# crowsonkb/style_transfer

Measured on AMD Instinct MI355X. Metric: tile-iterations/sec, VGG-19 2048px/1024-tile (fwd+bwd, Gram/content losses, regularizers, Adam step), higher is better.
Workload: dtype f32 (fp16x2-split MFMA, fp32 accumulate)

## Files before the change

style_transfer_amd/csrc/common.h:

```cpp
#pragma once

#include <hip/hip_runtime.h>

#include <vector>

#include <cstdarg>
#include <cstdio>
#include <functional>
#include <string>

#include "stx.h"

namespace stx {

constexpr float kEps = 1.1920928955078125e-07f;

void set_error(const char *fmt, ...);

const char *sw_env(const char *name);
void sw_reread();

#define STX_HIP(call)                                                                       \
    do {                                                                                    \
        hipError_t err__ = (call);                                                          \
// ... 175 lines not shown
    unsigned char *pool_codes;
    int skip_y = 0;
    unsigned char *out_codes = nullptr;
    unsigned char *in_codes = nullptr;
    const unsigned char *mask_codes = nullptr;
    long long *clock_out = nullptr;
    int item_base = 0;
    const unsigned *x_amax = nullptr;
    unsigned *y_amax = nullptr;
    const unsigned char *pin_codes = nullptr;
    int pin_mode = 0, pin_mask = 0;
#ifdef STX_EXPERIMENT_BF3
    int vp_rows = 0, vp_tp = 0;
#endif
};

bool conv_first_usable(int K, int M, int ksize);
int conv_first_workgroups(int H, int W);
int conv_first_launch(hipStream_t s, const float *x, const float *w_caffe, const float *bias, float *y,
                      int K, int H, int W, int relu, float *gram_partials, unsigned *y_amax = nullptr);

ConvConfig wino2_config(int geometry = 0);
int wino2_pick_geometry(int H, int W);
size_t wino2_packed_floats(int K, int M);
int wino2_pack_weights(hipStream_t s, const float *w_caffe, int Mo, int Ko, int transpose_flip,
                       float *packed);
int wino2_launch(hipStream_t s, const ConvConfig &cfg, const ConvProblem &p, int ksplit);
bool wino2_fuses_pool(const ConvProblem &p);
bool wino2_uses_relu_codes(const ConvProblem &p, int ksplit);
bool wino2_writes_out_codes(const ConvConfig &cfg, const ConvProblem &p);
int wino2_splitk_factor(const ConvConfig &cfg, const ConvProblem &p);
struct Wino2Tail { int items, slices; };
Wino2Tail wino2_tail_split(const ConvConfig &cfg, const ConvProblem &p);
int wino2_max_slices(const ConvConfig &cfg, const ConvProblem &p);

constexpr int kAmaxSlots = 64;
ConvConfig h2_config(int mb, int pb = 1);
ConvConfig h2_pick_config(const ConvProblem &p);
bool h2_usable(const ConvProblem &p);
size_t h2_packed_floats(int K, int M);
int h2_pack_weights(hipStream_t s, const float *w_caffe, int Mo, int Ko, int transpose_flip, float *packed);
int h2_launch(hipStream_t s, const ConvConfig &cfg, const ConvProblem &p, int ksplit);
int h2_splitk_factor(const ConvConfig &cfg, const ConvProblem &p);
bool h2_fuses_pool(const ConvProblem &p);
bool h2_takes_pooled_input(const ConvConfig &cfg, const ConvProblem &p);
int absmax_launch(hipStream_t s, const float *x, size_t n, unsigned *slots);

size_t conv_small_packed_floats(int K);
int conv_small_pack(hipStream_t s, const float *w_caffe, int Mo, int Ko, int transpose_flip,
                    float *packed);
int conv_small_launch(hipStream_t s, const float *x, const float *packed, float *y,
                      const float *mask, int K, int M, int H, int W);

bool conv_h2_enabled();
struct ConvTuner { int device; hipStream_t stream; hipEvent_t ev0, ev1; std::function<int(const ConvConfig &, const float **)> bank; };
int conv_choose(const ConvProblem &p, bool winograd, const ConvTuner *tuner, ConvConfig *out);
struct ConvBank { int key; size_t floats; std::function<int(hipStream_t, const float *w_caffe, float *packed)> pack; };
ConvBank conv_bank(const ConvConfig &cfg, int dir, int Mo, int Ko, int ksize);
ConvBank conv_small_bank(int Mo, int Ko);
int conv_dispatch(hipStream_t s, const ConvConfig &cfg, const ConvProblem &p, double *flop_algorithmic,
                  double *flop_issued);
int conv_splitk_factor(const ConvConfig &cfg, const ConvProblem &p);
size_t conv_splitk_floats(const ConvConfig &cfg, const ConvProblem &p);
bool conv_takes_clock(const ConvConfig &cfg);
bool conv_fuses_pool(const ConvConfig &cfg, const ConvProblem &p);
bool conv_writes_pool_codes(const ConvConfig &cfg);
bool conv_reads_x_amax(const ConvConfig &cfg);
bool conv_leaves_y_amax(const ConvConfig &cfg);
bool conv_takes_inject(const ConvConfig &cfg);
bool conv_takes_pooled_input(const ConvConfig &cfg, const ConvProblem &p);
bool conv_uses_relu_codes(const ConvConfig &cfg, const ConvProblem &p, int ksplit);
bool conv_writes_out_codes(const ConvConfig &cfg, const ConvProblem &p, int ksplit);

int pool_forward_launch(hipStream_t s, const float *x, int C, int H, int W, int mode, float *y,
                        unsigned char *codes = nullptr);
int pool_backward_codes_launch(hipStream_t s, const float *dy, const unsigned char *codes, int C,
                               int H, int W, int mode, bool relu_mask, float *dx);
int pool_backward_launch(hipStream_t s, const float *dy, const float *x, int C, int H, int W,
                         int mode, bool relu_mask, float *dx);

struct GramPlan {
    int C, HW, splits, tiles;
    int parts;
    size_t partial_floats;
};
GramPlan gram_plan(int C, int HW);
bool gram_h2_usable(const float *feat, int C, int HW);
int gram_partials_launch(hipStream_t s, const float *feat, const GramPlan &plan, float *partials,
                         const unsigned *f_amax = nullptr);
int gram_finish_blocks(const GramPlan &plan);
int gram_finish_launch(hipStream_t s, const float *partials, const GramPlan &plan, float *gram_out,
                       const float *target, float *dsym, float *sumsq, unsigned short *pieces = nullptr,
                       const unsigned *f_amax = nullptr, float *block_out = nullptr);

size_t symm_pieces_elems(int C);
int symm_num_workgroups(int C, int HW);
bool symm_bf3_usable(const float *feat, const float *out, int C, int HW);
bool symm_h2_usable(const float *feat, const float *out, int C, int HW);
int symm_h2_launch(hipStream_t s, const float *feat, const float *dsym, const unsigned *d_amax, int n_damax,
                   const unsigned *f_amax, float *out, float *partials, int C, int HW);
int symm_bf3_launch(hipStream_t s, const float *feat, const float *dsym, unsigned short *pieces,
                    bool pieces_ready, float *out, float *partials, int C, int HW);

#ifdef __HIPCC__
__device__ __forceinline__ int content_origin_y(const ContentWindow &w) { return w.oy - w.sy; }
__device__ __forceinline__ int content_origin_x(const ContentWindow &w) { return w.ox - w.sx; }
__device__ __forceinline__ size_t content_index(const ContentWindow &w, int c, int y, int x) {
    int yy = (content_origin_y(w) + y) % w.ch;
    int xx = (content_origin_x(w) + x) % w.cw;
    if (yy < 0) yy += w.ch;
    if (xx < 0) xx += w.cw;
    return ((size_t)c * w.ch + yy) * w.cw + xx;
}
#endif

struct SumJob {
    const float *src;
    int n;
    float *dst;
};
int sum_jobs_launch(hipStream_t s, const SumJob *jobs, int n_jobs);
int content_sums_launch(hipStream_t s, const float *feat, const float *content,
                        const ContentWindow &win, float *sums , std::vector<SumJob> *defer = nullptr);
int inject_style_launch(hipStream_t s, float *diff, const float *sgrad, size_t n,
                        const float *abs_sum, float coef, bool accumulate, unsigned *y_amax = nullptr);
int inject_content_launch(hipStream_t s, float *diff, const float *feat, const float *content,
                          const ContentWindow &win, const float *sums, float coef, bool accumulate,
                          unsigned *y_amax = nullptr);
int relu_inplace_launch(hipStream_t s, float *x, size_t n);
int sum_partials_launch(hipStream_t s, const float *partials, int n, float *out);
int sum_partials2_launch(hipStream_t s, const float *a, int na, float *out_a, const float *b, int nb,
                         float *out_b);

constexpr int kMaskParts = 1024;
constexpr int kMaskSgradParts = 2048;
int mask_map_launch(hipStream_t s, const float *mask, int H, int W, int scale, float *out);
int mask_apply_launch(hipStream_t s, const float *feat, const float *map, const ContentWindow &win, float *fm,
                      float *m2_partials, int *n_parts);
int mask_target_launch(hipStream_t s, const float *gs, int C, const float *m2_partials, int n_parts, int HW,
                       float *out, float *a_out);
int mask_sgrad_launch(hipStream_t s, float *sgrad, const float *map, const ContentWindow &win, const float *a,
                      float *partials, int *n_parts);

constexpr int kContentMaskParts = 1024;
int content_mask_mean_launch(hipStream_t s, const float *map, const ContentWindow &win, float *a_out);
int content_mask_term_launch(hipStream_t s, const float *feat, const float *content, const float *map,
                             const ContentWindow &win, const float *a, float *sgrad, float *partials,
                             int *n_parts);

constexpr int kStatSlice = 16384;
constexpr float kStatEps = 1e-5f;
int stat_slices(int HW);
size_t stat_scratch_floats(int C, int HW);
int stat_partials_launch(hipStream_t s, const float *feat, int C, int HW, float *partials);
int stat_finish_launch(hipStream_t s, const float *partials, int C, int HW, const float *MU, const float *SD,
                       float *table, float *e_out, float *mean_out, float *sd_out);
int stat_grad_launch(hipStream_t s, const float *feat, int C, int HW, const float *table, float *sgrad,
                     float *abs_partials, int *n_parts);

constexpr int kNnfmQ = 128, kNnfmB = 128, kNnfmK = 32, kNnfmMaxSlices = 64;
constexpr int kNnfmMaxK = 4;
struct NnfmPlan {
    int q_blocks, b_blocks, slices, blocks_per_slice;
};
NnfmPlan nnfm_plan(int n, int M);
size_t nnfm_pieces_floats(int rows, int C);
// ... 99 lines not shown
```

style_transfer_amd/csrc/gram.hip:

```cpp

#include <algorithm>
#include <cstdlib>
#include <cstring>

#include "bf16x3.h"
#include "common.h"
#include "f16x2.h"

namespace stx {

typedef float f32x16 __attribute__((ext_vector_type(16)));

constexpr int kGT = 64;
constexpr int kGP = 64;
constexpr int kGLd = kGP + 1;

GramPlan gram_plan(int C, int HW) {
    GramPlan p;
    p.C = C;
    p.HW = HW;
    const int T = ceil_div(C, kGT);
    p.tiles = T * (T + 1) / 2;
    int target = 512, min_stages = 8;
    if (const char *env = sw_env("STX_GRAM_WGS")) target = std::max(1, atoi(env));
    if (const char *env = sw_env("STX_GRAM_MIN_STAGES")) min_stages = std::max(1, atoi(env));
    int splits = std::max(1, target / p.tiles);
    splits = std::min(splits, ceil_div(HW, min_stages * kGP));
    splits = std::max(splits, 1);
    p.splits = splits;
    p.parts = 1;
    p.partial_floats = (size_t)p.splits * p.parts * p.tiles * kGT * kGT;
    return p;
}

__device__ __forceinline__ void tile_coords(int tile, int &ti, int &tj) {
    int r = (int)((sqrtf(8.f * tile + 1.f) - 1.f) * 0.5f);
    while ((r + 1) * (r + 2) / 2 <= tile) ++r;
    while (r * (r + 1) / 2 > tile) --r;
    ti = r;
    tj = tile - r * (r + 1) / 2;
}

template <bool VEC4>
__global__ __launch_bounds__(256, 2) void gram_partial_kernel(const float *__restrict__ F, int C,
                                                              int HW, int tiles, int slice,
                                                              int parts,
                                                              float *__restrict__ partials) {
    __shared__ float At[kGT * kGLd];
    __shared__ float Bt[kGT * kGLd];
    const int tid = threadIdx.x, lane = tid & 63;
    const int wave = __builtin_amdgcn_readfirstlane(tid >> 6);
    const int l31 = lane & 31, half = lane >> 5;
    const int tile = blockIdx.x % tiles, split = blockIdx.x / tiles;
    int ti, tj;
    tile_coords(tile, ti, tj);
    const bool diag = ti == tj;
    const int p_begin = split * slice;
    const int p_end = min(HW, p_begin + slice);
    const int bi = wave >> 1, bj = wave & 1;

    f32x16 acc;
#pragma unroll
    for (int r = 0; r < 16; ++r) acc[r] = 0.f;

    float ra[16], rb[16];
    auto load = [&](int p0) {
        if (VEC4) {
#pragma unroll
            for (int n = 0; n < 4; ++n) {
                const int e = tid + 256 * n;
                const int ch = e >> 4, px = p0 + (e & 15) * 4;
                const int ca = ti * kGT + ch, cb = tj * kGT + ch;
                const bool okp = px < p_end;
                const bool oka = okp && ca < C, okb = okp && cb < C && !diag;
                const float4 va = *reinterpret_cast<const float4 *>(F + (oka ? (size_t)ca * HW + px : 0));
                const float4 vb = *reinterpret_cast<const float4 *>(F + (okb ? (size_t)cb * HW + px : 0));
                ra[4 * n + 0] = oka ? va.x : 0.f;
                ra[4 * n + 1] = oka ? va.y : 0.f;
                ra[4 * n + 2] = oka ? va.z : 0.f;
                ra[4 * n + 3] = oka ? va.w : 0.f;
                rb[4 * n + 0] = okb ? vb.x : 0.f;
                rb[4 * n + 1] = okb ? vb.y : 0.f;
                rb[4 * n + 2] = okb ? vb.z : 0.f;
                rb[4 * n + 3] = okb ? vb.w : 0.f;
            }
        } else {
#pragma unroll
            for (int n = 0; n < 16; ++n) {
                const int e = tid + 256 * n;
                const int ch = e >> 6, px = p0 + (e & 63);
                const int ca = ti * kGT + ch, cb = tj * kGT + ch;
                const bool okp = px < p_end;
                const bool oka = okp && ca < C, okb = okp && cb < C && !diag;
                const float va = F[oka ? (size_t)ca * HW + px : 0];
                const float vb = F[okb ? (size_t)cb * HW + px : 0];
                ra[n] = oka ? va : 0.f;
                rb[n] = okb ? vb : 0.f;
            }
        }
    };
    auto store = [&]() {
        if (VEC4) {
#pragma unroll
            for (int n = 0; n < 4; ++n) {
                const int e = tid + 256 * n;
                const int ch = e >> 4, px = (e & 15) * 4;
#pragma unroll
                for (int k = 0; k < 4; ++k) {
                    At[ch * kGLd + px + k] = ra[4 * n + k];
                    if (!diag) Bt[ch * kGLd + px + k] = rb[4 * n + k];
                }
// ... 372 lines not shown
        }
    };
    auto store = [&](int p0, int buf) {
        float *At = lds + buf * kStageFloats, *Bt = At + kGT * kGLdW;
#pragma unroll
        for (int n = 0; n < 4; ++n) {
            const int rem = p_end - (p0 + ((tid + 256 * n) & 15) * 4);
            u32x4g va = ra[n], vb = rb[n];
            if (rem < 4) {
                va.x = rem > 0 ? va.x : 0u, va.y = rem > 1 ? va.y : 0u, va.z = rem > 2 ? va.z : 0u, va.w = 0u;
                vb.x = rem > 0 ? vb.x : 0u, vb.y = rem > 1 ? vb.y : 0u, vb.z = rem > 2 ? vb.z : 0u, vb.w = 0u;
            }
            *reinterpret_cast<u32x4g *>(At + ldst[n]) = va;
            if (!diag) *reinterpret_cast<u32x4g *>(Bt + ldst[n]) = vb;
        }
    };

    const int a_off = l31 * kGLdW + wave * 16 + half * 8;
    const int b_off = (diag ? 0 : kGT * kGLdW) + a_off;
    const float sv = pow2f(h2_scale_exp(amax_of_slots(f_amax, kAmaxSlots)));
    auto fragment = [&](const float *q, f16x8h &hi, f16x8h &lo) {
        const f32x4g v0 = *reinterpret_cast<const f32x4g *>(q);
        const f32x4g v1 = *reinterpret_cast<const f32x4g *>(q + 4);
        const float x[8] = {v0.x, v0.y, v0.z, v0.w, v1.x, v1.y, v1.z, v1.w};
        split2_f16(x, sv, hi, lo);
    };

    if (p_begin < p_end) {
        load(p_begin);
        store(p_begin, 0);
        if (p_begin + kGP < p_end) load(p_begin + kGP);
        __syncthreads();
        int buf = 0;
        for (int p0 = p_begin; p0 < p_end; p0 += kGP, buf ^= 1) {
            const float *base = lds + buf * kStageFloats;
            f16x8h ah[2], al[2], bh[2], bl[2];
            fragment(base + a_off, ah[0], al[0]);
            fragment(base + a_off + 32 * kGLdW, ah[1], al[1]);
            if (!diag) {
                fragment(base + b_off, bh[0], bl[0]);
                fragment(base + b_off + 32 * kGLdW, bh[1], bl[1]);
            }
            if (p0 + kGP < p_end) store(p0 + kGP, buf ^ 1);
            if (p0 + 2 * kGP < p_end) load(p0 + 2 * kGP);
#pragma unroll
            for (int i = 0; i < 2; ++i)
#pragma unroll
                for (int j = 0; j < 2; ++j) {
                    if (diag && j > i) continue;
                    acc[i][j] = mfma_split3(ah[i], al[i], diag ? ah[j] : bh[j], diag ? al[j] : bl[j], acc[i][j]);
                }
            __syncthreads();
        }
    }
    float *red = lds + wave * (kGT * kGT);
#pragma unroll
    for (int i = 0; i < 2; ++i)
#pragma unroll
        for (int j = 0; j < 2; ++j)
#pragma unroll
            for (int r = 0; r < 16; ++r) {
                const int row = i * 32 + (r & 3) + 8 * (r >> 2) + 4 * half;
                red[row * kGT + j * 32 + l31] = acc[i][j][r];
            }
    __syncthreads();
    static_assert(4 * kGT * kGT <= 2 * kStageFloats, "the four partial tiles must fit the stage buffers");
    float *out = partials + ((size_t)split * tiles + tile) * (kGT * kGT);
#pragma unroll
    for (int n = 0; n < 4; ++n) {
        const int e = tid + 256 * n;
        const float4 w0 = reinterpret_cast<const float4 *>(lds)[e];
        const float4 w1 = reinterpret_cast<const float4 *>(lds + kGT * kGT)[e];
        const float4 w2 = reinterpret_cast<const float4 *>(lds + 2 * kGT * kGT)[e];
        const float4 w3 = reinterpret_cast<const float4 *>(lds + 3 * kGT * kGT)[e];
        float4 v;
        v.x = ((w0.x + w1.x) + w2.x) + w3.x;
        v.y = ((w0.y + w1.y) + w2.y) + w3.y;
        v.z = ((w0.z + w1.z) + w2.z) + w3.z;
        v.w = ((w0.w + w1.w) + w2.w) + w3.w;
        reinterpret_cast<float4 *>(out)[e] = v;
    }
}

static bool gram_use_bf3() {
    const char *env = sw_env("STX_GRAM");
    return !(env && !strcmp(env, "fp32"));
}

bool gram_h2_usable(const float *feat, int C, int HW) {
    const char *env = sw_env("STX_GRAM");
    if (env && (!strcmp(env, "fp32") || !strcmp(env, "bf3"))) return false;
    return (reinterpret_cast<uintptr_t>(feat) & 3) == 0 && 4.0 * C * (double)HW < 2147483648.0;
}

int gram_partials_launch(hipStream_t s, const float *feat, const GramPlan &plan, float *partials,
                         const unsigned *f_amax) {
    int slice = ceil_div(plan.HW, plan.splits);
    slice = ceil_div(slice, kGP) * kGP;
    const bool aligned = (reinterpret_cast<uintptr_t>(feat) & 15) == 0;
    const double bytes = 4.0 * plan.C * (double)plan.HW;
    if (f_amax) {
        gram_partial_h2_kernel<<<plan.tiles * plan.splits, 256, 0, s>>>(
            feat, plan.C, plan.HW, plan.tiles, slice, (unsigned)bytes, f_amax, partials);
        STX_CHECK_LAUNCH();
        return STX_OK;
    }
    if ((reinterpret_cast<uintptr_t>(feat) & 3) == 0 && bytes < 2147483648.0 && gram_use_bf3()) {
        gram_partial_bf3_kernel<<<plan.tiles * plan.splits, 256, 0, s>>>(
            feat, plan.C, plan.HW, plan.tiles, slice, (unsigned)bytes, partials);
        STX_CHECK_LAUNCH();
        return STX_OK;
    }
    if ((reinterpret_cast<uintptr_t>(feat) & 3) == 0 && bytes < 2147483648.0 && !sw_env("STX_GRAM_NARROW")) {
        gram_partial_wide_kernel<<<plan.tiles * plan.splits, 256, 0, s>>>(
            feat, plan.C, plan.HW, plan.tiles, slice, (unsigned)bytes, partials);
        STX_CHECK_LAUNCH();
        return STX_OK;
    }
    if (plan.parts > 1)
        STX_HIP(hipMemsetAsync(partials, 0, plan.partial_floats * sizeof(float), s));
    if (plan.HW % 4 == 0 && aligned)
        gram_partial_kernel<true><<<plan.tiles * plan.splits, 256, 0, s>>>(
            feat, plan.C, plan.HW, plan.tiles, slice, plan.parts, partials);
    else
        gram_partial_kernel<false><<<plan.tiles * plan.splits, 256, 0, s>>>(
            feat, plan.C, plan.HW, plan.tiles, slice, plan.parts, partials);
    STX_CHECK_LAUNCH();
    return STX_OK;
}

__global__ __launch_bounds__(256) void gram_finish_kernel(const float *__restrict__ partials, int C,
                                                          int tiles, int splits, float scale,
                                                          float *__restrict__ gram,
                                                          const float *__restrict__ target,
                                                          float *__restrict__ dsym,
                                                          float *__restrict__ block_sumsq,
                                                          unsigned short *__restrict__ pieces,
                                                          const unsigned *__restrict__ f_amax,
                                                          unsigned *__restrict__ block_amax) {
    __shared__ float lane_sum[4][64];
    __shared__ float red[64];
    __shared__ float redm[64];
    float unscale = 1.f;
    if (f_amax) unscale = pow2f(-h2_scale_exp(amax_of_slots(f_amax, kAmaxSlots)));
    const int el = threadIdx.x & 63, sl = threadIdx.x >> 6;
    const int idx = blockIdx.x * 64 + el;
    const bool valid = idx < C * C;
    int i = 0, j = 0;
    float sum = 0.f;
    if (valid) {
        i = idx / C;
        j = idx % C;
    }
    const bool lower = valid && i >= j;
    if (lower) {
        const int ti = i / kGT, tj = j / kGT;
        const int tile = ti * (ti + 1) / 2 + tj;
        const size_t stride = (size_t)tiles * (kGT * kGT);
        const float *p = partials + (size_t)tile * (kGT * kGT) + (i % kGT) * kGT + (j % kGT);
        float s0 = 0.f, s1 = 0.f, s2 = 0.f, s3 = 0.f;
        int s = sl;
        for (; s + 12 < splits; s += 16) {
            s0 += p[(size_t)s * stride];
            s1 += p[(size_t)(s + 4) * stride];
            s2 += p[(size_t)(s + 8) * stride];
            s3 += p[(size_t)(s + 12) * stride];
        }
        for (; s < splits; s += 4) s0 += p[(size_t)s * stride];
        sum = (s0 + s1) + (s2 + s3);
    }
    lane_sum[sl][el] = sum;
    __syncthreads();
    float sq = 0.f, dmax = 0.f;
    if (sl == 0 && valid) {
        if (lower) {
            const float g = ((((lane_sum[0][el] + lane_sum[1][el]) + (lane_sum[2][el] + lane_sum[3][el])) *
                              unscale) * unscale) * scale;
            if (gram) gram[idx] = g;
            if (target) {
                const float d = g - target[i * C + j];
                dsym[idx] = d;
                if (i != j) dsym[j * C + i] = d;
                if (pieces) {
// ... 126 lines not shown
```

style_transfer_amd/csrc/symm.hip:

```cpp

#include <algorithm>
#include <cstdlib>
#include <cstring>

#include "bf16x3.h"
#include "common.h"
#include "f16x2.h"

#ifndef STX_SYMM_SKIP
#define STX_SYMM_SKIP 0
#endif

namespace stx {

namespace {

constexpr int kSM = 64;
constexpr int kSN = 256;
#ifndef STX_SYMM_KSK
#define STX_SYMM_KSK 32
#endif
constexpr int kSK = STX_SYMM_KSK;
constexpr int kSPC = kSK / 16;
constexpr int kSegs = kSK / 8;
// ... 283 lines not shown
    auto d_store = [&](int buf) {
#pragma unroll
        for (int n = 0; n < kHDLoads; ++n) {
            unsigned h[2], l[2];
            const unsigned d0 = dreg[n].x, d1 = dreg[n].y, d2 = dreg[n].z, d3 = dreg[n].w;
            split2_f16_quad(__builtin_bit_cast(float, d0), __builtin_bit_cast(float, d1),
                            __builtin_bit_cast(float, d2), __builtin_bit_cast(float, d3), sd, h, l);
            typedef unsigned u32x2s __attribute__((ext_vector_type(2)));
            unsigned char *q = lds + buf * kHChunkBytes + ddst[n];
            *reinterpret_cast<u32x2s *>(q) = (u32x2s){h[0], h[1]};
            *reinterpret_cast<u32x2s *>(q + kPieceBytes) = (u32x2s){l[0], l[1]};
        }
    };
    d_store(0);
    if (n_chunks > 1) d_load(1);
    __syncthreads();

    const unsigned a_off = (unsigned)(l31 * kRowBytes + g * 16);
    auto do_step = [&](int slot_, int buf, int s_in_chunk) {
        f16x8h bh[2], bl[2], ah[2], al[2];
#pragma unroll
        for (int j = 0; j < 2; ++j) split2_f16(raw[slot_][j], sf, bh[j], bl[j]);
        const unsigned char *base = lds + buf * kHChunkBytes + a_off + s_in_chunk * 32;
#pragma unroll
        for (int i = 0; i < 2; ++i) {
            ah[i] = *reinterpret_cast<const f16x8h *>(base + i * 32 * kRowBytes);
            al[i] = *reinterpret_cast<const f16x8h *>(base + kPieceBytes + i * 32 * kRowBytes);
        }
#pragma unroll
        for (int i = 0; i < 2; ++i)
#pragma unroll
            for (int j = 0; j < 2; ++j) acc[i][j] = mfma_split3(ah[i], al[i], bh[j], bl[j], acc[i][j]);
    };

    int step = 0;
    auto advance = [&](int slot_) {
        const int chunk = step / kSPC, s_in = step % kSPC, buf = chunk & 1;
        if (step + kRing - 1 < n_steps) f_load(step + kRing - 1, (slot_ + kRing - 1) % kRing);
        do_step(slot_, buf, s_in);
        if (s_in == kSPC - 1) {
            if (chunk + 1 < n_chunks) d_store(buf ^ 1);
            if (chunk + 2 < n_chunks) d_load(chunk + 2);
            __syncthreads();
        }
        ++step;
    };
    while (step < n_steps) {
#pragma unroll
        for (int r = 0; r < kRing; ++r)
            if (step < n_steps) advance(r);
    }

    const float ud = pow2f(-ed), uf = pow2f(-ef);
    float asum = 0.f;
#pragma unroll
    for (int i = 0; i < 2; ++i)
#pragma unroll
        for (int r = 0; r < 16; ++r) {
            const int row = m0 + i * 32 + (r & 3) + 8 * (r >> 2) + 4 * g;
            const int row0 = min(__builtin_amdgcn_readfirstlane(m0 + i * 32 + (r & 3) + 8 * (r >> 2)), C);
            const unsigned so = BIG ? 0u : (unsigned)row0 * HW4;
            const int rows_left = C - row0 < 5 ? C - row0 : 5;
            const __amdgpu_buffer_rsrc_t rrow =
                BIG ? __builtin_amdgcn_make_buffer_rsrc(S + (size_t)row0 * (size_t)HW, 0,
                                                        (rows_left > 0 ? rows_left : 0) * HW * 4, 0x00020000)
                    : rs;
#pragma unroll
            for (int j = 0; j < 2; ++j) {
                const int px = px0 + j * 32 + l31;
                const bool ok = row < C && px < HW;
                const float v = (acc[i][j][r] * ud) * uf;
                asum += ok ? fabsf(v) : 0.f;
                const unsigned vo = ok ? (unsigned)((4 * g) * HW + px) * 4u : kOob;
                __builtin_amdgcn_raw_buffer_store_b32(__builtin_bit_cast(unsigned, v), rrow, vo, so, 0);
            }
        }
#pragma unroll
    for (int off = 32; off > 0; off >>= 1) asum += __shfl_down(asum, off, 64);
    if (lane == 0) wave_sum[wave] = asum;
    __syncthreads();
    if (tid == 0) partials[blockIdx.x] = ((wave_sum[0] + wave_sum[1]) + wave_sum[2]) + wave_sum[3];
}

__global__ void symm_split_kernel(const float *__restrict__ dsym, int C, int Cp,
                                  unsigned short *__restrict__ pieces) {
    const int idx = blockIdx.x * blockDim.x + threadIdx.x;
    if (idx >= Cp * Cp) return;
    const int i = idx / Cp, j = idx - i * Cp;
    unsigned short s1 = 0, s2 = 0, s3 = 0;
    if (i < C && j < C) split3_bf16_scalar(dsym[i * C + j], s1, s2, s3);
    pieces[idx] = s1;
    pieces[(size_t)Cp * Cp + idx] = s2;
    pieces[2 * (size_t)Cp * Cp + idx] = s3;
}

int symm_num_workgroups(int C, int HW) { return ceil_div(C, kSM) * ceil_div(HW, kSN); }

bool symm_bf3_usable(const float *feat, const float *out, int C, int HW) {
    const char *env = sw_env("STX_SYMM");
    if (env && !strcmp(env, "fp32")) return false;
    return 64.0 * (double)HW < 2147483648.0 &&
           ((reinterpret_cast<uintptr_t>(feat) | reinterpret_cast<uintptr_t>(out)) & 3) == 0;
}

int symm_bf3_launch(hipStream_t s, const float *feat, const float *dsym, unsigned short *pieces,
                    bool pieces_ready, float *out, float *partials, int C, int HW) {
    const int Cp = ceil_div(C, kSM) * kSM;
    if (!pieces_ready || Cp != C) {
        symm_split_kernel<<<ceil_div(Cp * Cp, 256), 256, 0, s>>>(dsym, C, Cp, pieces);
        STX_CHECK_LAUNCH();
    }
    const int m_tiles = Cp / kSM;
    const double bytes = 4.0 * C * (double)HW;
    const char *force_big = sw_env("STX_WINO_BIG");
    if (bytes >= 2147483648.0 || (force_big && atoi(force_big) == 1))
        symm_bf3_kernel<true><<<symm_num_workgroups(C, HW), 256, 0, s>>>(feat, pieces, out, partials, C, Cp,
                                                                       HW, 0u, m_tiles);
    else
        symm_bf3_kernel<false><<<symm_num_workgroups(C, HW), 256, 0, s>>>(feat, pieces, out, partials, C, Cp,
                                                                        HW, (unsigned)bytes, m_tiles);
    STX_CHECK_LAUNCH();
    return STX_OK;
}

bool symm_h2_usable(const float *feat, const float *out, int C, int HW) {
    const char *env = sw_env("STX_SYMM");
    if (env && (!strcmp(env, "fp32") || !strcmp(env, "bf3"))) return false;
    return C % 4 == 0 && symm_bf3_usable(feat, out, C, HW);
}

int symm_h2_launch(hipStream_t s, const float *feat, const float *dsym, const unsigned *d_amax, int n_damax,
                   const unsigned *f_amax, float *out, float *partials, int C, int HW) {
    const int Cp = ceil_div(C, kSM) * kSM;
    const int m_tiles = Cp / kSM;
    const double bytes = 4.0 * C * (double)HW;
    const char *force_big = sw_env("STX_WINO_BIG");
    if (bytes >= 2147483648.0 || (force_big && atoi(force_big) == 1))
        symm_h2_kernel<true><<<symm_num_workgroups(C, HW), 256, 0, s>>>(feat, dsym, d_amax, n_damax, f_amax, out,
                                                                      partials, C, Cp, HW, 0u, m_tiles);
    else
        symm_h2_kernel<false><<<symm_num_workgroups(C, HW), 256, 0, s>>>(feat, dsym, d_amax, n_damax, f_amax, out,
                                                                       partials, C, Cp, HW, (unsigned)bytes, m_tiles);
    STX_CHECK_LAUNCH();
    return STX_OK;
}

}
```

Before: 272.7.

## Add 128-row tiled variants of Gram partial and symmetric-multiply h2 kernels

Adds a 128x128-block Gram partial kernel (512 threads, dynamic LDS, diagonal-aware MFMA skipping) that stays opt-in through STX_GRAM=h2_128. It also adds a 128-row symm h2 kernel that is on by default when C>=256 and enough workgroups exist. Larger M tiles let each loaded feature fragment feed more MFMAs, which cuts global and LDS traffic per flop. The cost is more registers and fewer workgroups, which can lower occupancy, and the symm partials indexing is remapped so it stays compatible with the 64-row layout.

Result: no change. 272.1 (-0.2%).

```diff
diff --git a/style_transfer_amd/csrc/common.h b/style_transfer_amd/csrc/common.h
--- a/style_transfer_amd/csrc/common.h
+++ b/style_transfer_amd/csrc/common.h
@@ -281,6 +281,7 @@
 struct GramPlan {
     int C, HW, splits, tiles;
     int parts;
+    bool m128 = false;
     size_t partial_floats;
 };
 GramPlan gram_plan(int C, int HW);
diff --git a/style_transfer_amd/csrc/gram.hip b/style_transfer_amd/csrc/gram.hip
--- a/style_transfer_amd/csrc/gram.hip
+++ b/style_transfer_amd/csrc/gram.hip
@@ -14,6 +14,11 @@
 constexpr int kGT = 64;
 constexpr int kGP = 64;
 constexpr int kGLd = kGP + 1;
+
+static bool gram_m128_shape(int C, int HW) {
+    const char *env = sw_env("STX_GRAM");
+    return env && !strcmp(env, "h2_128") && C % 128 == 0 && 4.0 * C * (double)HW < 2147483648.0;
+}
 
 GramPlan gram_plan(int C, int HW) {
     GramPlan p;
@@ -21,12 +26,16 @@
     p.HW = HW;
     const int T = ceil_div(C, kGT);
     p.tiles = T * (T + 1) / 2;
-    int target = 512, min_stages = 8;
-    if (const char *env = sw_env("STX_GRAM_WGS")) target = std::max(1, atoi(env));
+    int target = 512, target128 = 256, min_stages = 8;
+    if (const char *env = sw_env("STX_GRAM_WGS")) target = target128 = std::max(1, atoi(env));
     if (const char *env = sw_env("STX_GRAM_MIN_STAGES")) min_stages = std::max(1, atoi(env));
-    int splits = std::max(1, target / p.tiles);
+    p.m128 = gram_m128_shape(C, HW);
+    if (p.m128) target = target128;
+    const int T2 = C / 128;
+    int splits = std::max(1, target / (p.m128 ? T2 * (T2 + 1) / 2 : p.tiles));
     splits = std::min(splits, ceil_div(HW, min_stages * kGP));
     splits = std::max(splits, 1);
+    if (p.m128) splits = ceil_div(HW, ceil_div(ceil_div(HW, splits), kGP) * kGP);
     p.splits = splits;
     p.parts = 1;
     p.partial_floats = (size_t)p.splits * p.parts * p.tiles * kGT * kGT;
@@ -565,6 +574,164 @@
     }
 }
 
+constexpr int kGT2 = 128;
+constexpr int kStage2Floats = 2 * kGT2 * kGLdW;
+constexpr size_t kGram128LdsBytes = 2 * kStage2Floats * sizeof(float);
+static_assert(8 * kGT * kGT <= 2 * kStage2Floats, "eight partial sub-tiles must fit the stage buffers");
+
+__global__ __launch_bounds__(512, 1) void gram_partial_h2_m128_kernel(const float *__restrict__ F, int C, int HW,
+                                                                      int tiles, int blocks, int slice,
+                                                                      unsigned f_bytes,
+                                                                      const unsigned *__restrict__ f_amax,
+                                                                      float *__restrict__ partials) {
+    extern __shared__ __attribute__((aligned(16))) float lds2[];
+    const int tid = threadIdx.x, lane = tid & 63;
+    const int wave = __builtin_amdgcn_readfirstlane(tid >> 6);
+    const int q = wave & 3, h = wave >> 2;
+    const int l31 = lane & 31, half = lane >> 5;
+    const int nb = gridDim.x, xcd = blockIdx.x & 7, slot = blockIdx.x >> 3;
+    const int q8 = nb >> 3, r8 = nb & 7;
+    const int L = (xcd < r8 ? xcd * (q8 + 1) : r8 * (q8 + 1) + (xcd - r8) * q8) + slot;
+    const int block = L % blocks, split = L / blocks;
+    int bi, bj;
+    tile_coords(block, bi, bj);
+    bi = __builtin_amdgcn_readfirstlane(bi);
+    bj = __builtin_amdgcn_readfirstlane(bj);
+    const bool diag = bi == bj;
+    const int p_begin = split * slice;
+    const int p_end = min(HW, p_begin + slice);
+
+    f32x16 acc[2][2][2];
+#pragma unroll
+    for (int b = 0; b < 2; ++b)
+#pragma unroll
+        for (int i = 0; i < 2; ++i)
+#pragma unroll
+            for (int j = 0; j < 2; ++j)
+#pragma unroll
+                for (int r = 0; r < 16; ++r) acc[b][i][j][r] = 0.f;
+
+    const __amdgpu_buffer_rsrc_t rf =
+        __builtin_amdgcn_make_buffer_rsrc(const_cast<float *>(F), 0, f_bytes, 0x00020000);
+    unsigned aoff[4], boff[4];
+    int ldst[4];
+#pragma unroll
+    for (int n = 0; n < 4; ++n) {
+        const int e = tid + 512 * n;
+        const int ch = e >> 4, px = (e & 15) * 4;
+        aoff[n] = (unsigned)((bi * kGT2 + ch) * HW + px) * 4u;
+        boff[n] = (unsigned)((bj * kGT2 + ch) * HW + px) * 4u;
+        ldst[n] = ch * kGLdW + px;
+    }
+    u32x4g ra[4], rb[4];
+    auto load = [&](int p0) {
+        const unsigned so = (unsigned)__builtin_amdgcn_readfirstlane(p0 * 4);
+#pragma unroll
+        for (int n = 0; n < 4; ++n) ra[n] = __builtin_amdgcn_raw_buffer_load_b128(rf, aoff[n], so, 0);
+        if (!diag) {
+#pragma unroll
+            for (int n = 0; n < 4; ++n) rb[n] = __builtin_amdgcn_raw_buffer_load_b128(rf, boff[n], so, 0);
+        }
+    };
+    auto store = [&](int p0, int buf) {
+        float *At = lds2 + buf * kStage2Floats, *Bt = At + kGT2 * kGLdW;
+#pragma unroll
+        for (int n = 0; n < 4; ++n) {
+            const int rem = p_end - (p0 + ((tid + 512 * n) & 15) * 4);
+            u32x4g va = ra[n], vb = rb[n];
+            if (rem < 4) {
+                va.x = rem > 0 ? va.x : 0u, va.y = rem > 1 ? va.y : 0u, va.z = rem > 2 ? va.z : 0u, va.w = 0u;
+                vb.x = rem > 0 ? vb.x : 0u, vb.y = rem > 1 ? vb.y : 0u, vb.z = rem > 2 ? vb.z : 0u, vb.w = 0u;
+            }
+            *reinterpret_cast<u32x4g *>(At + ldst[n]) = va;
+            if (!diag) *reinterpret_cast<u32x4g *>(Bt + ldst[n]) = vb;
+        }
+    };
+
+    const int f_off = l31 * kGLdW + q * 16 + half * 8;
+    const int a_off = h * kGT * kGLdW + f_off;
+    const int b_off = (diag ? 0 : kGT2 * kGLdW) + f_off;
+    const float sv = pow2f(h2_scale_exp(amax_of_slots(f_amax, kAmaxSlots)));
+    auto fragment = [&](const float *p, f16x8h &hi, f16x8h &lo) {
+        const f32x4g v0 = *reinterpret_cast<const f32x4g *>(p);
+        const f32x4g v1 = *reinterpret_cast<const f32x4g *>(p + 4);
+        const float x[8] = {v0.x, v0.y, v0.z, v0.w, v1.x, v1.y, v1.z, v1.w};
+        split2_f16(x, sv, hi, lo);
+    };
+    const bool skip1 = diag && h == 0;
+
+    if (p_begin < p_end) {
+        load(p_begin);
+        store(p_begin, 0);
+        if (p_begin + kGP < p_end) load(p_begin + kGP);
+        __syncthreads();
+        int buf = 0;
+        for (int p0 = p_begin; p0 < p_end; p0 += kGP, buf ^= 1) {
+            const float *base = lds2 + buf * kStage2Floats;
+            f16x8h ah[2], al[2], bh[2], bl[2];
+            fragment(base + a_off, ah[0], al[0]);
+            fragment(base + a_off + 32 * kGLdW, ah[1], al[1]);
+            fragment(base + b_off, bh[0], bl[0]);
+            fragment(base + b_off + 32 * kGLdW, bh[1], bl[1]);
+            if (p0 + kGP < p_end) store(p0 + kGP, buf ^ 1);
+            if (p0 + 2 * kGP < p_end) load(p0 + 2 * kGP);
+#pragma unroll
+            for (int i = 0; i < 2; ++i)
+#pragma unroll
+                for (int j = 0; j < 2; ++j) {
+                    if (diag && h == 0 && j > i) continue;
+                    acc[0][i][j] = mfma_split3(ah[i], al[i], bh[j], bl[j], acc[0][i][j]);
+                }
+            if (!skip1) {
+                fragment(base + b_off + kGT * kGLdW, bh[0], bl[0]);
+                fragment(base + b_off + (kGT + 32) * kGLdW, bh[1], bl[1]);
+#pragma unroll
+                for (int i = 0; i < 2; ++i)
+#pragma unroll
+                    for (int j = 0; j < 2; ++j) {
+                        if (diag && j > i) continue;
+                        acc[1][i][j] = mfma_split3(ah[i], al[i], bh[j], bl[j], acc[1][i][j]);
+                    }
+            }
+            __syncthreads();
+        }
+    }
+#pragma unroll
+    for (int b = 0; b < 2; ++b) {
+        if (b) __syncthreads();
+        float *red = lds2 + (h * 4 + q) * (kGT * kGT);
+#pragma unroll
+        for (int i = 0; i < 2; ++i)
+#pragma unroll
+            for (int j = 0; j < 2; ++j)
+#pragma unroll
+                for (int r = 0; r < 16; ++r) {
+                    const int row = i * 32 + (r & 3) + 8 * (r >> 2) + 4 * half;
+                    red[row * kGT + j * 32 + l31] = acc[b][i][j][r];
+                }
+        __syncthreads();
+#pragma unroll
+        for (int n = 0; n < 4; ++n) {
+            const int e = tid + 512 * n;
+            const int hh = e >> 10, ee = e & 1023;
+            const int ti = 2 * bi + hh, tj = 2 * bj + b;
+            if (tj > ti) continue;
+            const float *w = lds2 + hh * 4 * (kGT * kGT);
+            const float4 w0 = reinterpret_cast<const float4 *>(w)[ee];
+            const float4 w1 = reinterpret_cast<const float4 *>(w + kGT * kGT)[ee];
+            const float4 w2 = reinterpret_cast<const float4 *>(w + 2 * kGT * kGT)[ee];
+            const float4 w3 = reinterpret_cast<const float4 *>(w + 3 * kGT * kGT)[ee];
+            float4 v;
+            v.x = ((w0.x + w1.x) + w2.x) + w3.x;
+            v.y = ((w0.y + w1.y) + w2.y) + w3.y;
+            v.z = ((w0.z + w1.z) + w2.z) + w3.z;
+            v.w = ((w0.w + w1.w) + w2.w) + w3.w;
+            float *out = partials + ((size_t)split * tiles + (ti * (ti + 1) / 2 + tj)) * (kGT * kGT);
+            reinterpret_cast<float4 *>(out)[ee] = v;
+        }
+    }
+}
+
 static bool gram_use_bf3() {
     const char *env = sw_env("STX_GRAM");
     return !(env && !strcmp(env, "fp32"));
@@ -582,6 +749,15 @@
     slice = ceil_div(slice, kGP) * kGP;
     const bool aligned = (reinterpret_cast<uintptr_t>(feat) & 15) == 0;
     const double bytes = 4.0 * plan.C * (double)plan.HW;
+    if (f_amax && plan.m128) {
+        const int T2 = plan.C / kGT2, blocks = T2 * (T2 + 1) / 2;
+        STX_HIP(hipFuncSetAttribute(reinterpret_cast<const void *>(gram_partial_h2_m128_kernel),
+                                    hipFuncAttributeMaxDynamicSharedMemorySize, (int)kGram128LdsBytes));
+        gram_partial_h2_m128_kernel<<<blocks * plan.splits, 512, kGram128LdsBytes, s>>>(
+            feat, plan.C, plan.HW, plan.tiles, blocks, slice, (unsigned)bytes, f_amax, partials);
+        STX_CHECK_LAUNCH();
+        return STX_OK;
+    }
     if (f_amax) {
         gram_partial_h2_kernel<<<plan.tiles * plan.splits, 256, 0, s>>>(
             feat, plan.C, plan.HW, plan.tiles, slice, (unsigned)bytes, f_amax, partials);
diff --git a/style_transfer_amd/csrc/symm.hip b/style_transfer_amd/csrc/symm.hip
--- a/style_transfer_amd/csrc/symm.hip
+++ b/style_transfer_amd/csrc/symm.hip
@@ -389,6 +389,184 @@
     if (tid == 0) partials[blockIdx.x] = ((wave_sum[0] + wave_sum[1]) + wave_sum[2]) + wave_sum[3];
 }
 
+constexpr int kSM2 = 128;
+constexpr int kPieceBytes2 = kSM2 * kRowBytes;
+constexpr int kHChunkBytes2 = 2 * kPieceBytes2;
+constexpr int kHDLoads2 = kSM2 * kSK / 4 / 256;
+
+__device__ __forceinline__ int symm_block_of_item(int L, int nb) {
+    const int q8 = nb >> 3, r8 = nb & 7, edge = r8 * (q8 + 1);
+    const int xcd = L < edge ? L / (q8 + 1) : r8 + (L - edge) / q8;
+    const int slot = L < edge ? L - xcd * (q8 + 1) : (L - edge) - (xcd - r8) * q8;
+    return slot * 8 + xcd;
+}
+
+__global__ __launch_bounds__(256, 2) void symm_h2_m128_kernel(const float *__restrict__ F,
+                                                              const float *__restrict__ D,
+                                                              const unsigned *__restrict__ d_amax, int n_damax,
+                                                              const unsigned *__restrict__ f_amax,
+                                                              float *__restrict__ S,
+                                                              float *__restrict__ partials, int C, int HW,
+                                                              unsigned f_bytes, int m_tiles) {
+    __shared__ __attribute__((aligned(16))) unsigned char lds[2 * kHChunkBytes2];
+    __shared__ float wave_sum[2][4];
+    __shared__ unsigned wave_max[4];
+    const int tid = threadIdx.x, lane = tid & 63;
+    const int wave = __builtin_amdgcn_readfirstlane(tid >> 6);
+    const int l31 = lane & 31, g = lane >> 5;
+    const int nb = gridDim.x, xcd = blockIdx.x & 7, slot = blockIdx.x >> 3;
+    const int q8 = nb >> 3, r8 = nb & 7;
+    const int L = (xcd < r8 ? xcd * (q8 + 1) : r8 * (q8 + 1) + (xcd - r8) * q8) + slot;
+    const int mt = __builtin_amdgcn_readfirstlane(L % m_tiles), pt = __builtin_amdgcn_readfirstlane(L / m_tiles);
+    const int m0 = mt * kSM2;
+    const int px0 = pt * kSN + wave * 64;
+
+    constexpr unsigned kOob = 0x80000000u;
+    const __amdgpu_buffer_rsrc_t rf = __builtin_amdgcn_make_buffer_rsrc(const_cast<float *>(F), 0, f_bytes, 0x00020000);
+    const __amdgpu_buffer_rsrc_t rs = __builtin_amdgcn_make_buffer_rsrc(S, 0, f_bytes, 0x00020000);
+    const __amdgpu_buffer_rsrc_t rd =
+        __builtin_amdgcn_make_buffer_rsrc(const_cast<float *>(D), 0, (unsigned)(C * C) * 4u, 0x00020000);
+    unsigned voff[2];
+#pragma unroll
+    for (int j = 0; j < 2; ++j) {
+        const int px = px0 + j * 32 + l31;
+        voff[j] = px < HW ? (unsigned)((g * 8) * HW + px) * 4u : kOob;
+    }
+    const unsigned HW4 = (unsigned)HW * 4u;
+    const int n_steps = C / 16, n_chunks = C / kSK;
+
+    unsigned dvoff[kHDLoads2], ddst[kHDLoads2];
+#pragma unroll
+    for (int n = 0; n < kHDLoads2; ++n) {
+        const int e = tid + 256 * n;
+        const int row = e / (kSK / 4), seg = e - row * (kSK / 4);
+        dvoff[n] = (unsigned)((m0 + row) * C + seg * 4) * 4u;
+        ddst[n] = (unsigned)(row * kRowBytes + seg * 8);
+    }
+    u32x4y dreg[kHDLoads2];
+    auto d_load = [&](int chunk) {
+        const unsigned so = (unsigned)__builtin_amdgcn_readfirstlane(chunk * kSK * 4);
+#pragma unroll
+        for (int n = 0; n < kHDLoads2; ++n) dreg[n] = __builtin_amdgcn_raw_buffer_load_b128(rd, dvoff[n], so, 0);
+    };
+
+    float raw[kRing][2][8];
+    auto f_load = [&](int step, int slot_) {
+        const int k0 = __builtin_amdgcn_readfirstlane(step * 16);
+#pragma unroll
+        for (int j = 0; j < 2; ++j)
+#pragma unroll
+            for (int e = 0; e < 8; ++e)
+                raw[slot_][j][e] = __builtin_bit_cast(
+                    float, __builtin_amdgcn_raw_buffer_load_b32(rf, voff[j], (unsigned)(k0 + e) * HW4, 0));
+    };
+
+    f32x16h acc[4][2];
+#pragma unroll
+    for (int i = 0; i < 4; ++i)
+#pragma unroll
+        for (int j = 0; j < 2; ++j)
+#pragma unroll
+            for (int r = 0; r < 16; ++r) acc[i][j][r] = 0.f;
+
+    d_load(0);
+#pragma unroll
+    for (int r = 0; r < kRing - 1; ++r)
+        if (r < n_steps) f_load(r, r);
+
+    const int ef = h2_scale_exp(amax_of_slots(f_amax, kAmaxSlots));
+    unsigned dm = 0;
+    for (int i = tid; i < n_damax; i += 256) dm = max(dm, d_amax[i]);
+#pragma unroll
+    for (int off = 32; off > 0; off >>= 1) dm = max(dm, (unsigned)__shfl_xor((int)dm, off, 64));
+    if (lane == 0) wave_max[wave] = dm;
+    __syncthreads();
+    dm = max(max(wave_max[0], wave_max[1]), max(wave_max[2], wave_max[3]));
+    const int ed = __builtin_amdgcn_readfirstlane(h2_scale_exp(dm));
+    const float sf = pow2f(ef), sd = pow2f(ed);
+
+    auto d_store = [&](int buf) {
+#pragma unroll
+        for (int n = 0; n < kHDLoads2; ++n) {
+            unsigned h[2], l[2];
+            const unsigned d0 = dreg[n].x, d1 = dreg[n].y, d2 = dreg[n].z, d3 = dreg[n].w;
+            split2_f16_quad(__builtin_bit_cast(float, d0), __builtin_bit_cast(float, d1),
+                            __builtin_bit_cast(float, d2), __builtin_bit_cast(float, d3), sd, h, l);
+            typedef unsigned u32x2s __attribute__((ext_vector_type(2)));
+            unsigned char *q = lds + buf * kHChunkBytes2 + ddst[n];
+            *reinterpret_cast<u32x2s *>(q) = (u32x2s){h[0], h[1]};
+            *reinterpret_cast<u32x2s *>(q + kPieceBytes2) = (u32x2s){l[0], l[1]};
+        }
+    };
+    d_store(0);
+    if (n_chunks > 1) d_load(1);
+    __syncthreads();
+
+    const unsigned a_off = (unsigned)(l31 * kRowBytes + g * 16);
+    auto do_step = [&](int slot_, int buf, int s_in_chunk) {
+        f16x8h bh[2], bl[2];
+#pragma unroll
+        for (int j = 0; j < 2; ++j) split2_f16(raw[slot_][j], sf, bh[j], bl[j]);
+        const unsigned char *base = lds + buf * kHChunkBytes2 + a_off + s_in_chunk * 32;
+#pragma unroll
+        for (int i = 0; i < 4; ++i) {
+            const f16x8h ah = *reinterpret_cast<const f16x8h *>(base + i * 32 * kRowBytes);
+            const f16x8h al = *reinterpret_cast<const f16x8h *>(base + kPieceBytes2 + i * 32 * kRowBytes);
+#pragma unroll
+            for (int j = 0; j < 2; ++j) acc[i][j] = mfma_split3(ah, al, bh[j], bl[j], acc[i][j]);
+        }
+    };
+
+    int step = 0;
+    auto advance = [&](int slot_) {
+        const int chunk = step / kSPC, s_in = step % kSPC, buf = chunk & 1;
+        if (step + kRing - 1 < n_steps) f_load(step + kRing - 1, (slot_ + kRing - 1) % kRing);
+        do_step(slot_, buf, s_in);
+        if (s_in == kSPC - 1) {
+            if (chunk + 1 < n_chunks) d_store(buf ^ 1);
+            if (chunk + 2 < n_chunks) d_load(chunk + 2);
+            __syncthreads();
+        }
+        ++step;
+    };
+    while (step < n_steps) {
+#pragma unroll
+        for (int r = 0; r < kRing; ++r)
+            if (step < n_steps) advance(r);
+    }
+
+    const float ud = pow2f(-ed), uf = pow2f(-ef);
+    float asum[2] = {0.f, 0.f};
+#pragma unroll
+    for (int i = 0; i < 4; ++i)
+#pragma unroll
+        for (int r = 0; r < 16; ++r) {
+            const int row0 = __builtin_amdgcn_readfirstlane(m0 + i * 32 + (r & 3) + 8 * (r >> 2));
+            const unsigned so = (unsigned)row0 * HW4;
+#pragma unroll
+            for (int j = 0; j < 2; ++j) {
+                const int px = px0 + j * 32 + l31;
+                const bool ok = px < HW;
+                const float v = (acc[i][j][r] * ud) * uf;
+                asum[i >> 1] += ok ? fabsf(v) : 0.f;
+                const unsigned vo = ok ? (unsigned)((4 * g) * HW + px) * 4u : kOob;
+                __builtin_amdgcn_raw_buffer_store_b32(__builtin_bit_cast(unsigned, v), rs, vo, so, 0);
+            }
+        }
+#pragma unroll
+    for (int u = 0; u < 2; ++u) {
+#pragma unroll
+        for (int off = 32; off > 0; off >>= 1) asum[u] += __shfl_down(asum[u], off, 64);
+        if (lane == 0) wave_sum[u][wave] = asum[u];
+    }
+    __syncthreads();
+    if (tid < 2) {
+        const int item = pt * (2 * m_tiles) + 2 * mt + tid;
+        partials[symm_block_of_item(item, 2 * nb)] =
+            ((wave_sum[tid][0] + wave_sum[tid][1]) + wave_sum[tid][2]) + wave_sum[tid][3];
+    }
+}
+
 __global__ void symm_split_kernel(const float *__restrict__ dsym, int C, int Cp,
                                   unsigned short *__restrict__ pieces) {
     const int idx = blockIdx.x * blockDim.x + threadIdx.x;
@@ -442,7 +620,18 @@
     const int m_tiles = Cp / kSM;
     const double bytes = 4.0 * C * (double)HW;
     const char *force_big = sw_env("STX_WINO_BIG");
-    if (bytes >= 2147483648.0 || (force_big && atoi(force_big) == 1))
+    const bool big = bytes >= 2147483648.0 || (force_big && atoi(force_big) == 1);
+    const char *env = sw_env("STX_SYMM");
+    const int wgs128 = (C / kSM2) * ceil_div(HW, kSN);
+    const bool want128 = env && !strcmp(env, "h2_128") ? true
+                         : env && !strcmp(env, "h2_64") ? false : C >= 256 && wgs128 >= 512;
+    if (!big && C % kSM2 == 0 && want128) {
+        symm_h2_m128_kernel<<<(C / kSM2) * ceil_div(HW, kSN), 256, 0, s>>>(feat, dsym, d_amax, n_damax, f_amax, out,
+                                                                           partials, C, HW, (unsigned)bytes, C / kSM2);
+        STX_CHECK_LAUNCH();
+        return STX_OK;
+    }
+    if (big)
         symm_h2_kernel<true><<<symm_num_workgroups(C, HW), 256, 0, s>>>(feat, dsym, d_amax, n_damax, f_amax, out,
                                                                       partials, C, Cp, HW, 0u, m_tiles);
     else
```
